# Nightmare-n/GD-MAE

Hardware: AMD Instinct MI355X
Metric: MAE pre-train frames/sec (Waymo-shape, 180k pts, 75% mask) (higher is better)
Workload: dtype bf16

## Files before the change

gd-mae_amd/csrc/decoder_blocks.hip:

```cpp
#include "../../include/gdmae_hip.h"
#include "common.h"
#include "dw_grouped.h"
#include <stdlib.h>

typedef float f32x16 __attribute__((ext_vector_type(16)));
typedef __bf16 bf16x8 __attribute__((ext_vector_type(8)));
typedef short s16x4 __attribute__((ext_vector_type(4)));

namespace {

constexpr int kC = 128;
constexpr int kChunk = 64;
constexpr int kXBytes = kChunk * kC * 2;
constexpr int kMaxTok = 2048;
constexpr int kHP = 6;
constexpr int kQ = 32;

template <int U>
struct Geo {
  static constexpr int TPC = kChunk / (U * U);
  static constexpr int HW = U + 2;
  static constexpr int HS = HW * HW;
  static constexpr int LT = U == 4 ? 36 : 24;
  static constexpr int NP = 2;
// ... 259 lines not shown

template <int U>
int block_dw_launch(const BlockDwArgs& A, hipStream_t st) {
  using G = Geo<U>;
  constexpr int lds = 2 * G::Buf + 3 * kC * 4 + kMaxTok * 16 + 3 * G::HRP * 4;
  static bool once = false;
  if (!once) {
    GD_CHECK(hipFuncSetAttribute((const void*)k_decoder_block_dw<U>, hipFuncAttributeMaxDynamicSharedMemorySize, lds));
    once = true;
  }
  hipLaunchKernelGGL((k_decoder_block_dw<U>), dim3(4u * (unsigned)A.S), dim3(512), lds, st, A);
  GD_LAUNCH_CHECK();
  return 0;
}

}

extern "C" size_t gdmae_decoder_block_dw_workspace_bytes(long long n, int u) {
  if (u != 2 && u != 4) return 0;
  if (n <= 0) return 256;
  int S = 0, cps = 0;
  block_dw_pick(n, &S, &cps);
  if (!block_dw_fits(u, cps)) return 0;
  return gd_align((size_t)S * 9 * kC * kC * sizeof(float));
}

extern "C" int gdmae_decoder_block_dw(const void* P, const float* a, const float* b, const void* bg, const int* site, long long n, int u,
                                      const void* dYc, const int* tile_slot, int H, int W, float* out, int ld_out, int m_off,
                                      void* workspace, void* stream) {
  GD_REQUIRE(u == 2 || u == 4, "decoder_block_dw: u must be 2 or 4");
// ... 18 lines not shown
```

gd-mae_amd/csrc/plan.hip:

```cpp
#include "../../include/gdmae_hip.h"
#include "common.h"
#include <string.h>

int gd_voxelize_impl(const float* points, long long n_points, int n_cols, const float* lo, const float* vs, const int* grid_xyz,
                     int batch_size, float* points_out, long long* point_coords, long long* inverse, int* inverse32,
                     long long* voxel_coords, int* pillar_cell, int* pillar_pt_off, int* pillar_pts, int* point_rank,
                     int* sample_pillar_off, float* pillar_mean, int* cell2pillar_out, int* counts, void* workspace, size_t workspace_bytes,
                     void* lb_state, float* points_pm, int* row_pillar, hipStream_t st);
size_t gd_voxelize_lb_state_bytes(long long n_points, long long cells);
size_t gd_plan_scan_state_bytes(long long n);
size_t gd_plan_win_state_bytes(long long n);
int gd_plan_visible_tokens(const float* mask, const int* cell2pillar, long long n_cells, int* tok_pillar, int* tok_cell, int* map,
                           int* n_tok, void* lb_state, hipStream_t st);
int gd_plan_downsample(const int* map_in, int B, int Yi, int Xi, int* tok_cell_out, int* map_out, int* n_out, void* lb_state,
                       hipStream_t st);
struct Dims {
  int B, Y, X;
};
struct PlanJob {
  const int* n_tok;
  const int* tok_cell;
  Dims dt, dm;
  const int* map;
  int mode, s;
// ... 176 lines not shown
    O.s[i].win_ws = L.add(name("win_ws"), gd_plan_windows_ws_bytes(B, g.Y, g.X, p->win_x[i], p->win_y[i]));
    const long long wcap = g.n_win < g.cap ? g.n_win : g.cap;
    for (int sh = 0; sh < 2; ++sh)
      for (int k = 0; k < 7; ++k) {
        snprintf(nm, sizeof(nm), "s%d.w%d.%s", i, sh, kWin[k]);
        O.s[i].w[sh][k] = L.add(nm, sizeof(int) * (k < 5 ? g.cap : wcap));
      }
  }
  O.dec_slot = O.dec_list = O.dec_flag = -1;
  if (O.dec) {
    O.dec_slot = L.add("dec.tile_slot", sizeof(int) * nt);
    O.dec_list = L.add("dec.tile_list", sizeof(int) * nt);
    O.dec_flag = L.add("dec.flag", sizeof(int) * nt);
    for (int g = 0; g < p->n_dec; ++g) {
      const StageGeo& sg = O.geo[p->dec_sources[g]];
      snprintf(nm, sizeof(nm), "dec.nbr%d", g);
      O.dec_nbr[g] = L.add(nm, sizeof(int) * sg.cap * sg.up_s * sg.up_s * 9);
    }
  }
  GD_REQUIRE(L.ok, "geometry plan: buffer table too small");
  if (total) *total = L.off;
  if (n_entries) *n_entries = L.n;
  return 0;
}

}

extern "C" int gdmae_geometry_plan_layout(const gdmae_plan_params* p, gdmae_plan_buffer* table, int max_entries, int* n_entries,
                                          size_t* total_bytes) {
  Offsets O;
// ... 89 lines not shown
    rc = gd_plan_windows_all(W, ns, st);
    if (rc) return rc;
  }
  if (O.dec) {
    const int* maps[3];
    int ups[3];
    for (int g = 0; g < p->n_dec; ++g) {
      maps[g] = I(O.s[p->dec_sources[g]].map);
      ups[g] = O.geo[p->dec_sources[g]].up_s;
    }
    int rc = gd_decoder_tiles_lb(maps, ups, p->n_dec, B, gy, gx, I(O.dec_slot), I(O.dec_list), n_act, I(O.dec_flag), lb, st);
    if (rc) return rc;
    for (int g = 0; g < p->n_dec; ++g) {
      const int si = p->dec_sources[g];
      const StageGeo& sg = O.geo[si];
      const int* sites = sg.up_s > 1 ? I(O.s[si].up_sites) : I(O.s[si].tok_cell);
      rc = gd_decoder_site_rulebook(sites, n_tok + si, sg.up_s * sg.up_s, sg.cap * sg.up_s * sg.up_s, I(O.dec_slot), gy, gx, I(O.dec_nbr[g]), st);
      if (rc) return rc;
    }
  }
  return 0;
}
```

gd-mae_amd/gdmae_hip/decoder.py:

```python
from __future__ import annotations

import os
from collections import namedtuple
from dataclasses import dataclass
from types import SimpleNamespace
from typing import Optional

import torch
import torch.nn.functional as F

from . import bn as gbn
from . import lib as L
from . import ops, packing
from . import plan as gplan
from . import timing

CONV_BWD = os.environ.get("GDMAE_DEC_BWD", "implicit")
BLOCK_BWD = os.environ.get("GDMAE_DEC_BLOCK", "1")



def colstats(x2d: torch.Tensor):
    R, C = x2d.shape
    assert x2d.is_contiguous() and x2d.dtype in (torch.float32, torch.bfloat16)
    out = torch.empty(2 * C, dtype=torch.float64, device=x2d.device)
    ws = torch.empty(L.load().gdmae_colstats_workspace_bytes(C), dtype=torch.uint8, device=x2d.device)
    L.call("gdmae_colstats", L.ptr(x2d), R, C, int(x2d.dtype == torch.bfloat16), L.ptr(out), L.ptr(ws), L.stream())
    return out[:C], out[C:]


def _gather_slice(table2d, idx, col0, ncol):
    es = table2d.element_size()
    out = torch.empty(idx.numel(), ncol, dtype=table2d.dtype, device=table2d.device)
# ... 123 lines not shown
    return _Forward(y2, yrows, stats2, ab2, mv2, Z, None, None, bgz)


def _backward_schedule(geom, conv_w, sites, Ps, widths, fwd):
    C2 = fwd.y2.shape[1]
    native = conv_w.dtype == torch.float32 and conv_w.is_contiguous() and C2 % 8 == 0
    tc = geom.tile_conv
    if not (CONV_BWD == "implicit" and fwd.tile_slot is not None and fwd.y2.dtype == torch.bfloat16 and native and C2 == 128
            and all(w == 128 for w in widths) and tc is not None):
        return native, ["taps"] * len(widths)
    stage_bwd = []
    for P, st, u in zip(Ps, sites, tc.ups):
        n, u = P.shape[0], int(u)
        block = (BLOCK_BWD != "0" and u in (2, 4) and P.dtype == torch.bfloat16 and P.is_contiguous() and st.numel() >= n
                 and int(L.load().gdmae_decoder_block_dw_workspace_bytes(n, u)) > 0)
        stage_bwd.append("block" if block else "rulebook")
    return native, stage_bwd


def _save(ctx, **named):
    ctx.saved_names = [(name, len(v) if isinstance(v, (list, tuple)) else None) for name, v in named.items()]
    ctx.save_for_backward(*[t for v in named.values() for t in (v if isinstance(v, (list, tuple)) else (v,))])


def _saved(ctx) -> SimpleNamespace:
    sv, out, j = ctx.saved_tensors, SimpleNamespace(), 0
    for name, n in ctx.saved_names:
        setattr(out, name, sv[j] if n is None else sv[j:j + n])
        j += 1 if n is None else n
    return out

# ... 50 lines not shown
    tot = torch.einsum('ko,koi->i', S, Wk.double()).contiguous()
    dWk = (S[:, :, None] * bgz.double()[None, None, :]).to(torch.promote_types(torch.float32, conv_w.dtype))
    Wd = Wk.to(cdt)
    return S, tot, dWk, Wd


def _stage_dx_spconv(b, i, col):
    n, w, C2 = b.Ps[i].shape[0], b.widths[i], b.y2.shape[1]
    nbr = b.tiles.nbr[i]
    assert nbr.shape[0] == n, (nbr.shape, n)
    dX = torch.empty(n, w, dtype=b.cdt, device=b.y2.device)
    L.call("gdmae_spconv", L.ptr(b.dYc), 0, L.ptr(nbr), b.packed.data_ptr() + i * 9 * w * C2 * 2, n, C2, w, L.ptr(dX), 8, L.stream())
    return dX


def _stage_grads_block(b, i, col):
    dX = _stage_dx_spconv(b, i, col)
    P, ab, w, u = b.Ps[i], b.ab_l[i], b.widths[i], int(b.ups[i])
    n = P.shape[0]
    ws = torch.empty(int(L.load().gdmae_decoder_block_dw_workspace_bytes(n, u)), dtype=torch.uint8, device=P.device)
    L.call("gdmae_decoder_block_dw", L.ptr(P), L.ptr(ab), L.ptr(ab[w:]), L.ptr(b.bgz[col:col + w]), L.ptr(b.sites[i]), n, u, L.ptr(b.dYc),
           L.ptr(b.tile_slot), b.H, b.W, L.ptr(b.dWk), b.bgz.numel(), col, L.ptr(ws), L.stream())
    return dX, None


def _stage_grads_rulebook(b, i, col):
    dX = _stage_dx_spconv(b, i, col)
    P, ab, w, C2 = b.Ps[i], b.ab_l[i], b.widths[i], b.y2.shape[1]
    n = P.shape[0]
    n_pad = int(L.load().gdmae_tap_dw_rows(n, w, C2))
    Zd = torch.empty(n_pad, w, dtype=b.cdt, device=P.device)
    L.call("gdmae_rows_affine_relu_sub", L.ptr(P), _bf(P), None, n, w, L.ptr(ab), L.ptr(ab[w:]), L.ptr(b.bgz[col:col + w]), L.ptr(Zd),
           _bf(Zd), w, 0, L.stream())
    ws = torch.empty(L.load().gdmae_tap_dw_workspace_bytes(n, w, C2), dtype=torch.uint8, device=P.device)
    L.call("gdmae_tap_dw", L.ptr(Zd), n, n_pad, w, L.ptr(b.dYc), L.ptr(b.tiles.nbr[i]), C2, L.ptr(b.dWk), b.bgz.numel(), col, L.ptr(ws),
           L.stream())
    return dX, None

# ... 4 lines not shown
    G = torch.empty(n, 9 * C2, dtype=cdt, device=dev)
    with timing.kernel("k_conv_grad_taps", 2.0 * n * 9 * C2 * G.element_size()):
        L.call("gdmae_conv3x3_grad_taps", L.ptr(b.y2), _bf(b.y2), L.ptr(b.tile_slot), L.ptr(b.ybg), L.ptr(b.k01), L.ptr(b.k01[C2:]),
               L.ptr(b.rows), L.ptr(b.cell2pillar), L.ptr(b.sites[i]), n, b.H, b.W, C2, L.ptr(G), L.stream())
    dX = ops.mm(G, b.Wd[:, :, col:col + w].reshape(9 * C2, w))
    bg = b.bgz[col:col + w]
    if b.Z is not None:
        Zd = _gather_slice(b.Z, b.sites[i], col, w) - bg
    else:
        Zd = torch.empty(n, w, dtype=cdt, device=dev)
        L.call("gdmae_rows_affine_relu_sub", L.ptr(P), _bf(P), None, n, w, L.ptr(ab), L.ptr(ab[w:]), L.ptr(bg), L.ptr(Zd),
               _bf(Zd), w, 0, L.stream())
    return dX, ops.splitk_tn(G, Zd)


_STAGE_GRADS = {"block": _stage_grads_block, "rulebook": _stage_grads_rulebook, "taps": _stage_grads_taps}


def _stage_bn_backward(b, i, col, dX, R, direct):
    P, ab, w = b.Ps[i], b.ab_l[i], b.widths[i]
    n = P.shape[0]
    ws = torch.empty(L.load().gdmae_rows_bwd_stats_workspace_bytes(w), dtype=torch.uint8, device=P.device)
    L.call("gdmae_rows_bwd_stats", L.ptr(P), _bf(P), None, n, w, L.ptr(ab), L.ptr(ab[w:]), L.ptr(dX), _bf(dX), w, 0,
           None, L.ptr(ws), L.stream())
    dgamma, dbeta, c01 = gbn.bwd_coeffs((ws, L.load().gdmae_rows_bwd_stats_rows(n)), 3, b.stats_l[i], ab, b.gammas[i], R,
                                        b.tot[col:col + w], direct)
    dP = torch.empty_like(P)
    L.call("gdmae_rows_bwd", L.ptr(P), _bf(P), None, n, w, L.ptr(ab), L.ptr(ab[w:]), L.ptr(c01), L.ptr(c01[w:]), L.ptr(dX),
           _bf(dX), w, 0, L.ptr(dP), _bf(dP), L.stream())
    return dP, dgamma, dbeta

# ... 41 lines not shown
        B, H, W = geom.B, geom.H, geom.W
        R, k = B * H * W, len(widths)
        b = _saved(ctx)
        b.H, b.W, b.cdt, b.widths = H, W, geom.cdt, widths
        b.rows, st2, b.k01, dgamma2, dbeta2 = _bn2_backward(b, dout, R, ctx.direct[k])
        reg = _region_sums(b, b.rows, B, H, W)
        tap_region, cnt = _region_consts(reg.device, B, H, W)
        algebra = region_algebra_native if ctx.native_region else region_algebra_torch
        S, b.tot, b.dWk, b.Wd = algebra(b.stats2, b.ab2, st2, b.k01, reg, tap_region, cnt, R, b.conv_w, b.bgz, geom.cdt)
        if stage_bwd[0] != "taps":
            b.packed = packing.decoder_conv_packed(ctx.conv_param, widths, ctx.direct_w is not None)
            if b.packed is None:
                stage_bwd = ["taps"] * k
            else:
                b.tiles, b.ups = geom.tile_conv.tiles, geom.tile_conv.ups
                if b.tiles.nbr is None:
                    b.tiles.nbr = gplan.decoder_site_rulebooks(b.tiles, b.sites, b.ups)
                C2 = b.y2.shape[1]
                b.dYc = torch.empty_like(b.y2)
                L.call("gdmae_decoder_dy", L.ptr(b.y2), L.ptr(b.tiles.tile_list), b.tiles.n_act, L.ptr(b.k01), L.ptr(b.k01[C2:]),
                       L.ptr(b.rows), L.ptr(b.cell2pillar), H, W, C2, L.ptr(b.dYc), L.stream())
        grads = [None] * 8
        dW_rows = []
        col = 0
        for i, w in enumerate(widths):
            dX, dW = _STAGE_GRADS[stage_bwd[i]](b, i, col)
            if dW is not None:
                dW_rows.append(dW)
            grads += [None, *_stage_bn_backward(b, i, col, dX, R, ctx.direct[i])]
            col += w
        dWk = b.dWk
        if dW_rows:
# ... 170 lines not shown
```

gd-mae_amd/gdmae_hip/lib.py:

```python
from __future__ import annotations

import ctypes as C
import os

import torch

_HERE = os.path.dirname(os.path.abspath(__file__))
LIB_PATH = os.path.abspath(os.path.join(_HERE, "..", "csrc", "libgdmae_hip.so"))
if os.environ.get("GDMAE_LIB"):
    LIB_PATH = os.path.abspath(os.environ["GDMAE_LIB"])


class GdmaeHipError(RuntimeError):
    pass


_P, _I, _L, _F, _D, _Z = C.c_void_p, C.c_int, C.c_longlong, C.c_float, C.c_double, C.c_size_t

SIGNATURES = {
    "gdmae_abi_version": (_I, []),
    "gdmae_target_arch": (C.c_char_p, []),
    "gdmae_last_error": (C.c_char_p, []),
    "gdmae_voxelize_workspace_bytes": (_Z, [_L, _I, _I, _I, _I]),
    "gdmae_voxelize": (_I, [_P, _L, _I, _P, _P, _P, _I, _P, _P, _P, _P, _P, _P, _P, _P, _P, _P, _P, _P, _P, _P, _Z, _P]),
# ... 94 lines not shown
    "gdmae_gemm_tn_splitk": (_I, [_P, _P, _P, _L, _I, _I, _I, _I, _P, _P]),
    "gdmae_conv_block_scratch_bytes": (_Z, [_L, _L, _I, _I, _I]),
    "gdmae_spconv_packed_bytes": (_Z, [_I, _I]),
    "gdmae_spconv_pack_jobs": (_I, [_P, _I, _I, _I, _P, _P]),
    "gdmae_spconv": (_I, [_P, _I, _P, _P, _L, _I, _I, _P, _I, _P]),
    "gdmae_spconv_bias_relu": (_I, [_P, _I, _P, _P, _P, _L, _I, _I, _P, _P]),
    "gdmae_spconv_stat_rows": (_I, [_I, _I, _I]),
    "gdmae_spconv_stats": (_I, [_P, _I, _P, _P, _L, _I, _I, _P, _P, _P]),
    "gdmae_decoder_dy": (_I, [_P, _P, _I, _P, _P, _P, _P, _I, _I, _I, _P, _P]),
    "gdmae_decoder_site_rulebook": (_I, [_P, _P, _I, _L, _P, _I, _I, _P, _P]),
    "gdmae_tap_dw_rows": (_L, [_L, _I, _I]),
    "gdmae_tap_dw_workspace_bytes": (_Z, [_L, _I, _I]),
    "gdmae_tap_dw": (_I, [_P, _L, _L, _I, _P, _P, _I, _P, _I, _I, _P, _P]),
    "gdmae_decoder_block_dw_workspace_bytes": (_Z, [_L, _I]),
    "gdmae_decoder_block_dw": (_I, [_P, _P, _P, _P, _P, _L, _I, _P, _P, _I, _I, _P, _I, _I, _P, _P]),
    "gdmae_conv_block_fwd": (_I, [_P, _P]),
    "gdmae_conv_block_bwd": (_I, [_P, _P]),
    "gdmae_encoder_layer_bytes": (_I, [_L, _I, _I, _I, _I, _P, _P, _P]),
    "gdmae_dw_gemm_workspace_bytes": (_Z, [_L, _I, _I]),
    "gdmae_dw_gemm": (_I, [_P, _P, _L, _I, _I, _P, _P, _P, _P]),
    "gdmae_layer_packed_bytes": (_Z, [_I, _I]),
    "gdmae_layer_pack_jobs": (_I, [_P, _P, _P, _P, _I, _I, _P, _P]),
    "gdmae_layer_pack_job_count": (_I, [_I, _I]),
    "gdmae_tok_gemm_pack": (_I, [_P, _I, _P]),
    "gdmae_tok_gemm": (_I, [_P, _P, _P, _L, _L, _I, _I, _I, _P, _P, _P, _P, _P, _P, _F, _P, _P, _P, _P, _P, _P, _P]),
    "gdmae_tok_gemm_qkv": (_I, [_P, _P, _P, _P, _P, _L, _I, _P, _P, _P]),
    "gdmae_tok_gemm_ffn": (_I, [_P, _P, _P, _P, _P, _L, _L, _I, _P, _P, _P, _P, _F, _P, _P, _P, _P, _P, _P, _P, _P]),
    "gdmae_tok_gemm_ln_bwd_rows": (_I, [_I]),
    "gdmae_tok_gemm_ln_bwd": (_I, [_P, _P, _L, _L, _I, _I, _P, _P, _P, _P, _P, _P, _P, _P, _P, _P]),
    "gdmae_encoder_layer_fwd": (_I, [_P, _P]),
# ... 69 lines not shown
}

class LayerArgs(C.Structure):
    _fields_ = ([("n", _L), ("d", _I), ("ff", _I), ("nhead", _I), ("bf16", _I), ("eps", _F), ("tau_min", _F), ("n_levels", _I),
                 ("n_win", _I * 4), ("max_tokens", _I * 4)]
                + [(k, _P) for k in ("tok_pos", "csr_tok", "win_start", "win_len", "pos_table", "Win", "bin", "Wo", "bo", "W1", "b1",
                                     "W2", "b2", "g1", "be1", "g2", "be2", "tau", "x", "y", "dy", "dx", "dWin", "dbin", "dtau", "dWo",
                                     "dbo", "dW1", "db1", "dW2", "db2", "dg1", "dbe1", "dg2", "dbe2", "saved", "scratch", "packed")]
                + [("x_bf16", _I), ("res_out", _P), ("dres", _P), ("dx_bf16", _P), ("path", _I)])


class PlanParams(C.Structure):
    _fields_ = [("n_points", _L), ("n_cols", _I), ("batch_size", _I), ("lo", _F * 3), ("vs", _F * 3), ("grid", _I * 3), ("n_stages", _I),
                ("stride", _I * 4), ("win_x", _I * 4), ("win_y", _I * 4), ("n_levels", _I * 4), ("drop_lo", (_I * 3) * 4),
                ("drop_hi", (_I * 3) * 4), ("max_tokens", (_I * 3) * 4), ("masked", _I), ("keep_frac", _D), ("n_dec", _I),
                ("dec_sources", _I * 4), ("want_pm", _I), ("cap_points", _L)]


class PlanBuffer(C.Structure):
    _fields_ = [("name", C.c_char * 40), ("offset", _L), ("bytes", _L)]


class ConvBlockArgs(C.Structure):
    _fields_ = ([("n_in", _L), ("n_out", _L), ("cin", _I), ("cout", _I), ("bf16", _I), ("x_f32", _I), ("g_f32", _I),
                 ("eps", _F), ("momentum", _F)]
                + [(k, _P) for k in ("x", "nbr", "nbr_t", "W", "gamma", "beta", "running_mean", "running_var", "num_batches", "cols",
                                     "y", "stats", "ab", "mv", "out", "g", "dx", "dW", "dgamma", "dbeta", "scratch", "packed_fwd", "packed_bwd")]
                + [("out_f32", _I)])


_lib = None
# ... 65 lines not shown
```

gd-mae_amd/gdmae_hip/plan.py:

```python
from __future__ import annotations

from dataclasses import dataclass, field
from typing import List, Optional

import torch

from . import lib as L

I32 = torch.int32


def _empty(n, dtype, dev):
    return torch.empty(int(n), dtype=dtype, device=dev)


@dataclass
class VoxelPlan:
    batch_size: int
    grid: tuple
    lo: tuple
    vs: tuple
    n_cols: int
    N: int
    M: int
# ... 149 lines not shown
    sources = tuple(int(v) for v in sources)
    dt = ep.dec_tiles
    if dt is not None and dt.sources == sources and dt.H == H and dt.W == W:
        return dt
    st = [ep.stages[i] for i in sources]
    B = st[0].B
    ups = [H // sp.Y for sp in st]
    assert all(sp.Y * u == H and sp.X * u == W for sp, u in zip(st, ups))
    r = _decoder_tiles_launch([sp.map for sp in st], ups, B, H, W, st[0].map.device)
    n = int(r["n_act"].item())
    ep.dec_tiles = DecoderTiles(sources, B, H, W, n, r["tile_slot"], r["tile_list"][:n])
    ep.dec_tiles.nbr = _site_rulebooks(ep.dec_tiles, st, ups)
    return ep.dec_tiles


def decoder_site_rulebooks(dt: "DecoderTiles", sites, ups, n_tok=None):
    out = []
    for g, (st, u) in enumerate(zip(sites, ups)):
        n_dev = torch.tensor([st.numel() // (u * u) if n_tok is None else n_tok[g]], dtype=I32, device=st.device)
        nbr = _empty(st.numel() * 9, I32, st.device)
        L.call("gdmae_decoder_site_rulebook", L.ptr(st.contiguous()), L.ptr(n_dev), u * u, st.numel(), L.ptr(dt.tile_slot), dt.H, dt.W,
               L.ptr(nbr), L.stream())
        out.append(nbr.view(-1, 9))
    return out


def _site_rulebooks(dt: "DecoderTiles", stages, ups):
    sites = (sp.tok_cell if u == 1 else (sp._up_sites[1] if getattr(sp, "_up_sites", None) is not None and sp._up_sites[0] == u
                                         else upsample_cells(sp.tok_cell, sp.Y, sp.X, u).reshape(-1).contiguous())
             for sp, u in zip(stages, ups))
    return decoder_site_rulebooks(dt, sites, ups, [sp.n_tok for sp in stages])


def _encoder_launch(vox, m_cap: int, strides, window_shapes, drop_infos, keep_frac, noise, dec_sources=None) -> dict:
    if isinstance(vox, dict):
        dev, grid, B = vox["src"].device, vox["grid"], vox["batch_size"]
        sample_off, pillar_cell, vcounts = vox["sample_off"], vox["pillar_cell"], vox["counts"]
    else:
        dev, grid, B = vox.points.device, vox.grid, vox.batch_size
# ... 123 lines not shown
    e = _encoder_launch(vox, vox.M, strides, window_shapes, drop_infos, keep_frac, noise, dec_sources)
    return _encoder_finalize(e, e["counts"].tolist(), vox.M)


import collections
import time as _time

EVENT_WAIT_S = 0.0

_PLAN_SHAPES = collections.OrderedDict()
_PLAN_SHAPES_MAX = 32
_PLAN_GRANULE = 16384
_PINNED = {}


def _plan_shape(n0, ncols, B, pcr, voxel_size, grid_size, strides, window_shapes, drop_infos, keep_frac, dec_sources):
    gx, gy, gz = (int(g) for g in grid_size)
    lo = tuple(float(v) for v in pcr[:3])
    vs = tuple(float(v) for v in voxel_size)
    drops = tuple(tuple(map(tuple, _drop_arrays(d))) for d in drop_infos)
    n_exact = n0
    n0 = max(1, (n0 + _PLAN_GRANULE - 1) // _PLAN_GRANULE) * _PLAN_GRANULE
    key = (n0, ncols, B, lo, vs, (gx, gy, gz), tuple(int(s) for s in strides), tuple(tuple(int(v) for v in w) for w in window_shapes),
           drops, None if keep_frac is None else float(keep_frac), None if dec_sources is None else tuple(int(i) for i in dec_sources))
    hit = _PLAN_SHAPES.get(key)
    if hit is not None:
        _PLAN_SHAPES.move_to_end(key)
        return hit
    del n_exact
    import ctypes as C
    ns = len(strides)
    assert gz == 1, "the SST backbone works on single-layer pillar grids (spt_backbone_mae.py:94)"
    assert 1 <= ns <= 4
    P = L.PlanParams()
    P.n_points, P.cap_points, P.n_cols, P.batch_size = n0, n0, ncols, B
    for i in range(3):
        P.lo[i], P.vs[i] = lo[i], vs[i]
        P.grid[i] = (gx, gy, gz)[i]
    P.n_stages = ns
# ... 10 lines not shown
        for l in range(len(dT)):
            P.drop_lo[i][l], P.drop_hi[i][l], P.max_tokens[i][l] = dlo[l], dhi[l], dT[l]
        cap_in = cap
        if int(strides[i]) > 1:
            assert int(strides[i]) == 2, "only the k3 s2 p1 strided sparse conv of the shipped configs is implemented"
            Y, X = (Y - 1) // 2 + 1, (X - 1) // 2 + 1
            cap = min(4 * cap, B * Y * X)
        us = gy // Y
        up_s = us if (us >= 1 and us * Y == gy and us * X == gx) else 0
        geo.append(dict(Y=Y, X=X, cap=cap, cap_in=cap_in, up_s=up_s, strided=int(strides[i]) > 1, T=list(dT)))
    P.masked = int(keep_frac is not None)
    P.keep_frac = float(keep_frac) if keep_frac is not None else 1.0
    P.n_dec = 0 if dec_sources is None else len(dec_sources)
    for g in range(P.n_dec):
        P.dec_sources[g] = int(dec_sources[g])
    P.want_pm = 1
    table = (L.PlanBuffer * 160)()
    n_ent, total = C.c_int(0), C.c_size_t(0)
    L.call("gdmae_geometry_plan_layout", C.byref(P), table, 160, C.byref(n_ent), C.byref(total))
    names = {table[i].name.decode(): (int(table[i].offset), int(table[i].bytes)) for i in range(n_ent.value)}
    hit = _PLAN_SHAPES[key] = (P, names, int(total.value), geo, m_cap, (lo, vs, (gx, gy, gz)))
    while len(_PLAN_SHAPES) > _PLAN_SHAPES_MAX:
        _PLAN_SHAPES.popitem(last=False)
    return hit


class _Arena:

    def __init__(self, raw, names):
        self.raw, self.names = raw, names
# ... 6 lines not shown
        off, _ = self.names[name]
        es = 8 if dtype == torch.int64 else 4
        strides, acc = [], 1
        for d in reversed(shape):
            strides.append(acc)
            acc *= int(d)
        return self.base[dtype].as_strided(tuple(int(d) for d in shape), tuple(reversed(strides)), off // es)


class PlanPrefetch:

    _side = {}
    _arena_bytes = {}

    def __init__(self, points, point_cloud_range, voxel_size, grid_size, batch_size, strides, window_shapes, drop_infos,
                 keep_frac=None, noise=None, ready=None, dec_sources=None):
        import ctypes as C
        assert points.is_cuda and points.dtype == torch.float32 and points.dim() == 2
        points = points.contiguous()
        dev = points.device
        main = torch.cuda.current_stream(dev)
        side = PlanPrefetch._side.setdefault(dev.index, torch.cuda.Stream(device=dev))
        side.wait_stream(main)
        if ready is not None:
            side.wait_event(ready)
        points.record_stream(side)
        if noise is not None:
            noise.record_stream(side)
        n0, ncols = points.shape
        P, names, total, geo, m_cap, _ = self.shape = _plan_shape(n0, ncols, int(batch_size), point_cloud_range, voxel_size, grid_size,
                                                                    strides, window_shapes, drop_infos, keep_frac, dec_sources)
        self.masked, self.dec_sources, self.batch_size, self.ncols = keep_frac is not None, dec_sources, int(batch_size), ncols
        with torch.cuda.stream(side):
            cap = PlanPrefetch._arena_bytes.get(dev.index, 0)
            if total > cap:
                cap = PlanPrefetch._arena_bytes[dev.index] = -(-total // (64 << 20)) * (64 << 20)
            raw = torch.empty(cap, dtype=torch.uint8, device=dev)
            if self.masked and noise is None:
                noise = torch.rand(m_cap, device=dev, dtype=torch.float32)
            if noise is not None:
                assert noise.dtype == torch.float32 and noise.numel() >= 1
                noise = noise.contiguous()
            Pc = L.PlanParams.from_buffer_copy(P)
            Pc.n_points = n0
            L.call("gdmae_geometry_plan", C.byref(Pc), L.ptr(points), None if noise is None else L.ptr(noise), L.ptr(raw), total, L.stream())
            self.arena = _Arena(raw, names)
# ... 47 lines not shown
                wpre = f"{pre}w{k}."
                wps.append(WindowPlan(V(wpre + "tok_win", i32, n), V(wpre + "tok_level", i32, n), V(wpre + "tok_slot", i32, n),
                                      V(wpre + "tok_pos", i32, n), V(wpre + "csr_tok", i32, n), V(wpre + "win_start", i32, nw),
                                      V(wpre + "win_len", i32, nw), [int(v) for v in wc[0:3]], [int(v) for v in wc[3:6]], list(g["T"])))
            n_prev = (int(c[2 + i - 1]) if i > 0 else n_vis) if g["strided"] else 0
            sp = StagePlan(B, g["Y"], g["X"], n, V(pre + "tok_cell", i32, n), V(pre + "map", i32, B * g["Y"] * g["X"]),
                           V(pre + "nbr_subm", i32, n, 9), V(pre + "nbr_down", i32, n, 9) if g["strided"] else None,
                           V(pre + "nbr_down_t", i32, n_prev, 9) if g["strided"] else None, wps)
            sp._nbr_subm_t = V(pre + "nbr_subm_t", i32, n, 9)
            sp._up_sites = (g["up_s"], V(pre + "up_sites", i32, n * g["up_s"] * g["up_s"])) if g["up_s"] > 1 else None
            stages.append(sp)
        dt = None
        if A.has("dec.tile_slot"):
            n_act = int(c[2 + ns + 16 * ns])
            nt = B * ((gy + 7) // 8) * ((gx + 7) // 8)
            nbrs = [V(f"dec.nbr{g}", i32, stages[int(si)].n_tok * geo[int(si)]["up_s"] ** 2, 9) for g, si in enumerate(self.dec_sources)]
            dt = DecoderTiles(tuple(int(i) for i in self.dec_sources), B, gy, gx, n_act, V("dec.tile_slot", i32, nt), V("dec.tile_list", i32, n_act),
                              nbrs)
        ep = EncoderPlan(V("mask", f32, M) if self.masked else None, V("tok_pillar", i32, stages[0].n_tok if not geo[0]["strided"] else n_vis),
                         stages, dt)
        self.arena = self.points = self.keep = None
        return vox, ep


def _tensors_of(obj):
    out = []
    if isinstance(obj, torch.Tensor):
        if obj.is_cuda:
            out.append(obj)
    elif isinstance(obj, dict):
        for v in obj.values():
# ... 6 lines not shown
```

gd-mae_amd/pcdet/models/backbones_3d/spt_backbone_mae.py:

```python
import torch
import torch.nn as nn

from .spt_backbone import SSTBlockV1, build_decoder, run_decoder, stage_plan_args
from ...utils.spconv_utils import SparseConvTensor
from gdmae_hip import decoder as gdec, ops, plan as gplan


def _only_the_pred_head_sees_the_gradient(pred) -> bool:
    fn = pred.grad_fn
    if fn is None or not type(fn).__name__.startswith('ViewBackward') or pred._backward_hooks or pred.retains_grad:
        return False
    nxt = [f for f, _ in fn.next_functions if f is not None]
    if len(nxt) != 1 or 'PredHeadFn' not in type(nxt[0]).__name__:
        return False
    return not getattr(nxt[0], '_tensor_pre_hooks', None) and not getattr(nxt[0], '_pre_hooks', None) and not getattr(nxt[0], '_retains_grad_hooks', None)


class _DeferredPlan:
    __slots__ = ("_mod", "_args", "_pf")

    def __init__(self, mod, args):
        self._mod, self._args, self._pf = mod, args, None

    def __call__(self):
# ... 75 lines not shown
                                              pre_conv_hook=hook)
        else:
            sf = run_decoder(self.model_cfg, self.decoder_deblocks, self.decoder_conv_out, hidden)
            assert sf.shape[0] == B and sf.shape[2] == Y and sf.shape[3] == X
            pyramid = ops.GatherUnique.apply(sf.permute(0, 2, 3, 1).reshape(B * Y * X, sf.shape[1]), vox.pillar_cell)
        src0 = self.model_cfg.FEATURES_SOURCE[0]
        batch_dict.update({'encoded_spconv_tensor': hidden[-1], 'encoded_spconv_tensor_stride': Y0 // hidden[-1].spatial_shape[0],
                           'multi_scale_3d_features': feats, 'multi_scale_3d_strides': strides, 'spatial_features': sf,
                           'spatial_features_stride': strides[src0] // self.model_cfg.FUSE_LAYER[src0].UPSAMPLE_STRIDE})
        batch_dict.update({'voxel_features': pyramid, 'voxel_coords': all_coords,
                           'voxel_shuffle_inds': torch.arange(all_coords.shape[0], device=all_coords.device)})
        self.forward_ret_dict = self.target_assigner(batch_dict)
        return batch_dict

    def prefetch_plan(self, points, batch_size, noise=None, ready=None):
        return gplan.PlanPrefetch(points, self.point_cloud_range, self.voxel_size, self.grid_size, int(batch_size),
                                  *stage_plan_args(self.model_cfg.SST_BLOCK_LIST), keep_frac=1 - self.mask_ratio, noise=noise,
                                  ready=ready, dec_sources=self._dec_sources())

    def prefetch_plan_under_decoder(self, points, batch_size, noise=None, ready=None):
        self._pre_conv_hook = d = _DeferredPlan(self, (points, batch_size, noise, ready))
        return d

    def _dec_sources(self):
        if self.decoder_impl != 'sparse' or self.decoder_conv_impl != 'tiles':
            return None
        return [int(src[-1]) - 1 for src in self.model_cfg.FEATURES_SOURCE]

    def target_assigner(self, batch_dict):
        vox = batch_dict['_gdmae_vox']
        gt = ops.group_gt_points(vox, self.mask_cfg.NUM_GT_POINTS)
        flat = gdec.pred_head(batch_dict['voxel_features'], self.decoder_pred)
        return {'pred_points': flat.view(vox.M, -1, 3), 'gt_points': gt, 'mask': batch_dict['voxel_mae_mask'],
# ... 2 lines not shown
```

include/gdmae_hip.h:

```cpp
#ifndef GDMAE_HIP_H
#define GDMAE_HIP_H

#include <stddef.h>
#include <stdint.h>

#ifdef __cplusplus
extern "C" {
#endif

int gdmae_abi_version(void);
const char* gdmae_target_arch(void);
const char* gdmae_last_error(void);

size_t gdmae_voxelize_workspace_bytes(long long n_points, int batch_size, int gx, int gy, int gz);
int gdmae_voxelize(const float* points, long long n_points, int n_cols, const float* lo, const float* vs,
                   const int* grid_xyz, int batch_size, float* points_out, long long* point_coords,
                   long long* inverse, int* inverse32, long long* voxel_coords, int* pillar_cell,
                   int* pillar_pt_off, int* pillar_pts, int* point_rank, int* sample_pillar_off,
                   float* pillar_mean, int* cell2pillar, int* counts, void* workspace, size_t workspace_bytes,
                   void* stream);

int gdmae_decorate_points(const float* points, const long long* point_coords, const int* inverse32,
                          const float* pillar_mean, long long N, int n_cols, const float* lo, const float* vs,
                          float* out, void* stream);
// ... 222 lines not shown
int gdmae_spconv_stat_rows(int cin, int cout, int x_f32);
int gdmae_spconv_stats(const void* X, int x_f32, const int* nbr, const void* packed, long long n, int cin, int cout, void* Y, float* part,
                       void* stream);
int gdmae_decoder_dy(const void* Yc, const int* tile_list, int n_act, const float* k0, const float* k1, const float* rows,
                     const int* cell2pillar, int H, int W, int C, void* dYc, void* stream);
int gdmae_decoder_site_rulebook(const int* site, const int* n_dev, int sites_per_tok, long long cap_sites, const int* tile_slot,
                                int H, int W, int* nbr, void* stream);
long long gdmae_tap_dw_rows(long long n, int M, int N);
size_t gdmae_tap_dw_workspace_bytes(long long n, int M, int N);
int gdmae_tap_dw(const void* G, long long n, long long n_pad, int M, const void* X, const int* nbr, int N, float* out, int ld_out,
                 int m_off, void* workspace, void* stream);
size_t gdmae_decoder_block_dw_workspace_bytes(long long n, int u);
int gdmae_decoder_block_dw(const void* P, const float* a, const float* b, const void* bg, const int* site, long long n, int u,
                           const void* dYc, const int* tile_slot, int H, int W, float* out, int ld_out, int m_off, void* workspace,
                           void* stream);
int gdmae_conv_block_fwd(const gdmae_conv_block_args* args , void* stream);
int gdmae_conv_block_bwd(const gdmae_conv_block_args* args , void* stream);

typedef struct gdmae_layer_args {
  long long n;
  int d, ff, nhead, bf16;
  float eps, tau_min;
  int n_levels;
  int n_win[4], max_tokens[4];
  const int* tok_pos;
  const int* csr_tok;
  const int* win_start;
  const int* win_len;
  const float* pos_table;
  const void *Win, *bin, *Wo, *bo, *W1, *b1, *W2, *b2;
// ... 110 lines not shown
  long long n_points;
  int n_cols, batch_size;
  float lo[3], vs[3];
  int grid[3];
  int n_stages;
  int stride[GDMAE_PLAN_MAX_STAGES];
  int win_x[GDMAE_PLAN_MAX_STAGES], win_y[GDMAE_PLAN_MAX_STAGES];
  int n_levels[GDMAE_PLAN_MAX_STAGES];
  int drop_lo[GDMAE_PLAN_MAX_STAGES][3], drop_hi[GDMAE_PLAN_MAX_STAGES][3], max_tokens[GDMAE_PLAN_MAX_STAGES][3];
  int masked;
  double keep_frac;
  int n_dec;
  int dec_sources[GDMAE_PLAN_MAX_STAGES];
  int want_pm;
  long long cap_points;
} gdmae_plan_params;
typedef struct gdmae_plan_buffer {
  char name[40];
  long long offset, bytes;
} gdmae_plan_buffer;
int gdmae_geometry_plan_layout(const gdmae_plan_params* p, gdmae_plan_buffer* table, int max_entries, int* n_entries,
                               size_t* total_bytes);
int gdmae_geometry_plan(const gdmae_plan_params* p, const float* points, const float* noise, void* arena, size_t arena_bytes,
                        void* stream);

size_t gdmae_center_head_targets_workspace_bytes(int B, int num_max_objs);
int gdmae_center_head_targets(const float* gt_boxes, int B, int n_max, int box_dim, const int* class_map, int n_class_total,
                              int n_cls, const float* pc_range , const float* voxel_size ,
                              float feature_map_stride, int fw, int fh, int num_max_objs, double gaussian_overlap, int min_radius,
                              float* heatmap, float* ret_boxes, long long* inds, long long* mask, void* workspace, void* stream);
// ... 109 lines not shown
```

Baseline: 1104.

## Add block-tiled decoder conv dX kernel and skip unneeded site rulebooks

Adds a new HIP kernel that computes the decoder 3x3 conv input gradient per block of tokens. It stages a halo of dY rows from the tile map into swizzled LDS and runs bf16 MFMA over the 9 taps, replacing the gather-based spconv dX path. Because this path no longer needs the per-site neighbour rulebook, the geometry plan can now skip building and allocating those rulebooks for u=2/4 stages. The trade-offs are halo reads of masked rows, tied to fixed tile shapes, and more plan-key complexity.

```diff
diff --git a/gd-mae_amd/csrc/decoder_blocks.hip b/gd-mae_amd/csrc/decoder_blocks.hip
--- a/gd-mae_amd/csrc/decoder_blocks.hip
+++ b/gd-mae_amd/csrc/decoder_blocks.hip
@@ -297,6 +297,217 @@
   return 0;
 }
 
+struct BlockDxArgs {
+  const unsigned short* dY;
+  const int* site;
+  const int* tile_slot;
+  const uint4* Wp;
+  unsigned short* dZ;
+  long long n;
+  int ntok, H, W, TH, TW;
+};
+
+union DxFrag {
+  uint4 q;
+  bf16x8 v;
+};
+
+template <int U>
+__device__ __forceinline__ int dx_swz(int tl, int hy, int hx) {
+  return U == 4 ? (((hy & 3) << 2) | (hx & 3)) : (((tl & 3) << 2) | ((hy & 1) << 1) | (hx & 1));
+}
+
+template <int U, int ROWS, int WAVES>
+__global__ __launch_bounds__(64 * WAVES, 2) void k_decoder_block_dx(BlockDxArgs A) {
+  constexpr int NTHR = 64 * WAVES;
+  constexpr int KS = kC / 16;
+  constexpr int MB = kC / 32;
+  constexpr int WPB = WAVES / MB;
+  constexpr int NPW = ROWS / 32 / WPB;
+  constexpr int HW = U + 2, HS = HW * HW;
+  constexpr int NT = ROWS / (U * U);
+  constexpr int NHR = NT * HS;
+  constexpr int NP = NHR * 16 / NTHR;
+  constexpr int NR = (NHR + NTHR - 1) / NTHR;
+  constexpr int SP = kC * 2 + 16;
+  static_assert(WPB >= 1 && NPW >= 1 && NPW * WPB * 32 == ROWS && NP * NTHR == NHR * 16 && ROWS * SP <= NHR * 256, "tile shape");
+  constexpr int RING = KS;
+  extern __shared__ __align__(16) unsigned char lds[];
+  int* rowidx = reinterpret_cast<int*>(lds + NHR * 256);
+  const int tid = threadIdx.x, lane = tid & 63, wv = tid >> 6;
+  const long long row0 = (long long)blockIdx.x * ROWS;
+  const long long tok0 = (long long)blockIdx.x * NT;
+  const int mb0 = wv / WPB;
+  const int nb0 = (wv % WPB) * NPW;
+
+  int sv[NR];
+#pragma unroll
+  for (int j = 0; j < NR; ++j) {
+    const int hr = tid + j * NTHR < NHR ? tid + j * NTHR : NHR - 1;
+    const long long tok = tok0 + hr / HS;
+    sv[j] = A.site[(tok < A.ntok ? tok : (long long)A.ntok - 1) * (U * U)];
+  }
+
+  const uint4* __restrict__ wp = A.Wp + (size_t)mb0 * 64 + lane;
+  DxFrag wr[RING];
+#pragma unroll
+  for (int ks = 0; ks < RING; ++ks) wr[ks].q = wp[(size_t)ks * MB * 64];
+
+  {
+    int slot[NR], loc[NR];
+#pragma unroll
+    for (int j = 0; j < NR; ++j) {
+      const int hr = tid + j * NTHR < NHR ? tid + j * NTHR : NHR - 1;
+      const int tl = hr / HS, rem = hr - tl * HS;
+      const int hy = rem / HW, hx = rem - hy * HW;
+      const int x0 = sv[j] % A.W, r = sv[j] / A.W;
+      const int y0 = r % A.H, bb = r / A.H;
+      const int yy = y0 + hy - 1, xx = x0 + hx - 1;
+      const bool in = tok0 + tl < A.ntok && yy >= 0 && yy < A.H && xx >= 0 && xx < A.W;
+      slot[j] = A.tile_slot[in ? (bb * A.TH + (yy >> 3)) * A.TW + (xx >> 3) : 0];
+      loc[j] = in ? (yy & 7) * 8 + (xx & 7) : -1;
+    }
+#pragma unroll
+    for (int j = 0; j < NR; ++j) {
+      const int hr = tid + j * NTHR < NHR ? tid + j * NTHR : NHR - 1;
+      rowidx[hr] = (loc[j] >= 0 && slot[j] >= 0) ? slot[j] * 64 + loc[j] : -1;
+    }
+  }
+  __syncthreads();
+
+  {
+    const int pc = tid & 15;
+    uint4 q[NP];
+    unsigned keep = 0u;
+#pragma unroll
+    for (int p = 0; p < NP; ++p) {
+      const int rix = rowidx[(p * NTHR + tid) >> 4];
+      const bool ok = rix >= 0;
+      keep |= ok ? 1u << p : 0u;
+      q[p] = *reinterpret_cast<const uint4*>(A.dY + (long long)(ok ? rix : 0) * kC + pc * 8);
+    }
+#pragma unroll
+    for (int p = 0; p < NP; ++p) {
+      const int hr = (p * NTHR + tid) >> 4;
+      const int tl = hr / HS, rem = hr - tl * HS;
+      const int hy = rem / HW, hx = rem - hy * HW;
+      const unsigned m = ((keep >> p) & 1u) ? 0xFFFFFFFFu : 0u;
+      uint4 v = q[p];
+      v.x &= m; v.y &= m; v.z &= m; v.w &= m;
+      *reinterpret_cast<uint4*>(lds + hr * 256 + ((pc ^ dx_swz<U>(tl, hy, hx)) << 4)) = v;
+    }
+  }
+  __syncthreads();
+
+  int tlb[NPW], hyc[NPW], hxc[NPW];
+#pragma unroll
+  for (int b = 0; b < NPW; ++b) {
+    const int r = (nb0 + b) * 32 + (lane & 31);
+    tlb[b] = r / (U * U);
+    hyc[b] = (r / U) % U + 1;
+    hxc[b] = r % U + 1;
+  }
+  const int hsel = lane >> 5;
+
+  f32x16 acc[NPW];
+#pragma unroll
+  for (int b = 0; b < NPW; ++b)
+#pragma unroll
+    for (int i = 0; i < 16; ++i) acc[b][i] = 0.f;
+
+  int rb[NPW], sw[NPW];
+  auto tap_rows = [&](int tap) {
+#pragma unroll
+    for (int b = 0; b < NPW; ++b) {
+      const int hy = hyc[b] + 1 - tap / 3, hx = hxc[b] + 1 - tap % 3;
+      rb[b] = (tlb[b] * HS + hy * HW + hx) * 256;
+      sw[b] = (dx_swz<U>(tlb[b], hy, hx) ^ hsel) << 4;
+    }
+  };
+  DxFrag sf[2][NPW];
+  tap_rows(0);
+#pragma unroll
+  for (int b = 0; b < NPW; ++b) sf[0][b].q = *reinterpret_cast<const uint4*>(lds + rb[b] + sw[b]);
+#pragma unroll
+  for (int tap = 0; tap < 9; ++tap) {
+#pragma unroll
+    for (int ks = 0; ks < KS; ++ks) {
+      const int g = tap * KS + ks;
+      if (ks + 1 < KS) {
+#pragma unroll
+        for (int b = 0; b < NPW; ++b) sf[(g + 1) & 1][b].q = *reinterpret_cast<const uint4*>(lds + rb[b] + (((ks + 1) * 32) ^ sw[b]));
+      } else if (tap < 8) {
+        tap_rows(tap + 1);
+#pragma unroll
+        for (int b = 0; b < NPW; ++b) sf[(g + 1) & 1][b].q = *reinterpret_cast<const uint4*>(lds + rb[b] + sw[b]);
+      }
+#pragma unroll
+      for (int b = 0; b < NPW; ++b) acc[b] = __builtin_amdgcn_mfma_f32_32x32x16_bf16(wr[g % RING].v, sf[g & 1][b].v, acc[b], 0, 0, 0);
+      if (g + RING < 9 * KS) wr[g % RING].q = wp[(size_t)(g + RING) * MB * 64];
+      __builtin_amdgcn_sched_barrier(0);
+    }
+  }
+  __syncthreads();
+
+  {
+    const int cb = mb0 * 32 + 4 * (lane >> 5);
+#pragma unroll
+    for (int b = 0; b < NPW; ++b) {
+      const int row = (nb0 + b) * 32 + (lane & 31);
+#pragma unroll
+      for (int q = 0; q < 4; ++q) {
+        uint2 o;
+        o.x = gd_pack_bf16(acc[b][4 * q], acc[b][4 * q + 1]);
+        o.y = gd_pack_bf16(acc[b][4 * q + 2], acc[b][4 * q + 3]);
+        *reinterpret_cast<uint2*>(lds + row * SP + (cb + 8 * q) * 2) = o;
+      }
+    }
+  }
+  __syncthreads();
+  {
+    constexpr int OCPR = kC / 8;
+    constexpr int ORPP = NTHR / OCPR;
+    const int c = tid % OCPR, r = tid / OCPR;
+#pragma unroll
+    for (int p = 0; p < ROWS / ORPP; ++p) {
+      const int rl = p * ORPP + r;
+      if (row0 + rl < A.n) *reinterpret_cast<uint4*>(A.dZ + (row0 + rl) * kC + c * 8) = *reinterpret_cast<const uint4*>(lds + rl * SP + c * 16);
+    }
+  }
+}
+
+template <int U, int ROWS, int WAVES>
+int block_dx_launch(const BlockDxArgs& A, hipStream_t st) {
+  constexpr int nhr = ROWS / (U * U) * (U + 2) * (U + 2);
+  constexpr int lds = nhr * 256 + nhr * 4;
+  static bool once = false;
+  if (!once) {
+    GD_CHECK(hipFuncSetAttribute((const void*)k_decoder_block_dx<U, ROWS, WAVES>, hipFuncAttributeMaxDynamicSharedMemorySize, lds));
+    once = true;
+  }
+  hipLaunchKernelGGL((k_decoder_block_dx<U, ROWS, WAVES>), dim3((unsigned)gd_div_up(A.n, ROWS)), dim3(64 * WAVES), lds, st, A);
+  GD_LAUNCH_CHECK();
+  return 0;
+}
+
+}
+
+extern "C" int gdmae_decoder_block_dx_supported(long long n, int u) {
+  return (u == 2 || u == 4) && n >= 0 && n % (u * u) == 0 && n < (1ll << 31);
+}
+
+extern "C" int gdmae_decoder_block_dx(const void* dYc, const int* site, long long n, int u, const int* tile_slot, int H, int W,
+                                      const void* packed, void* dZ, void* stream) {
+  GD_REQUIRE(u == 2 || u == 4, "decoder_block_dx: u must be 2 or 4");
+  GD_REQUIRE(n >= 0 && n % (u * u) == 0, "decoder_block_dx: rows must be whole tokens (u * u sites each)");
+  if (n == 0) return 0;
+  GD_REQUIRE(n < (1ll << 31) && H > 0 && W > 0 && H % u == 0 && W % u == 0, "decoder_block_dx: map size");
+  hipStream_t st = (hipStream_t)stream;
+  BlockDxArgs A{(const unsigned short*)dYc, site, tile_slot, (const uint4*)packed, (unsigned short*)dZ, n, (int)(n / (u * u)), H, W,
+                (H + 7) / 8, (W + 7) / 8};
+  GdTimed timed(GD_T_DEC_CONV_BWD, st, (double)n / (u * u) * ((u + 2) * (u + 2) * 2.0 * kC + 4.0) + (double)n * 2.0 * kC + 18.0 * kC * kC,
+                2.0 * n * 9.0 * kC * kC);
+  return u == 4 ? block_dx_launch<4, 128, 4>(A, st) : block_dx_launch<2, 64, 4>(A, st);
 }
 
 extern "C" size_t gdmae_decoder_block_dw_workspace_bytes(long long n, int u) {
diff --git a/gd-mae_amd/csrc/plan.hip b/gd-mae_amd/csrc/plan.hip
--- a/gd-mae_amd/csrc/plan.hip
+++ b/gd-mae_amd/csrc/plan.hip
@@ -214,6 +214,8 @@
     O.dec_flag = L.add("dec.flag", sizeof(int) * nt);
     for (int g = 0; g < p->n_dec; ++g) {
       const StageGeo& sg = O.geo[p->dec_sources[g]];
+      O.dec_nbr[g] = -1;
+      if (p->dec_skip_rulebook[g]) continue;
       snprintf(nm, sizeof(nm), "dec.nbr%d", g);
       O.dec_nbr[g] = L.add(nm, sizeof(int) * sg.cap * sg.up_s * sg.up_s * 9);
     }
@@ -333,6 +335,7 @@
     for (int g = 0; g < p->n_dec; ++g) {
       const int si = p->dec_sources[g];
       const StageGeo& sg = O.geo[si];
+      if (O.dec_nbr[g] < 0) continue;
       const int* sites = sg.up_s > 1 ? I(O.s[si].up_sites) : I(O.s[si].tok_cell);
       rc = gd_decoder_site_rulebook(sites, n_tok + si, sg.up_s * sg.up_s, sg.cap * sg.up_s * sg.up_s, I(O.dec_slot), gy, gx, I(O.dec_nbr[g]), st);
       if (rc) return rc;
diff --git a/gd-mae_amd/gdmae_hip/decoder.py b/gd-mae_amd/gdmae_hip/decoder.py
--- a/gd-mae_amd/gdmae_hip/decoder.py
+++ b/gd-mae_amd/gdmae_hip/decoder.py
@@ -17,6 +17,12 @@
 
 CONV_BWD = os.environ.get("GDMAE_DEC_BWD", "implicit")
 BLOCK_BWD = os.environ.get("GDMAE_DEC_BLOCK", "1")
+BLOCK_DX = os.environ.get("GDMAE_DEC_BLOCK_DX", "1")
+
+
+def plan_rulebooks(ups):
+    blocks = CONV_BWD == "implicit" and BLOCK_BWD != "0" and BLOCK_DX != "0"
+    return [not (blocks and int(u) in (2, 4)) for u in ups]
 
 
 
@@ -170,7 +176,9 @@
         n, u = P.shape[0], int(u)
         block = (BLOCK_BWD != "0" and u in (2, 4) and P.dtype == torch.bfloat16 and P.is_contiguous() and st.numel() >= n
                  and int(L.load().gdmae_decoder_block_dw_workspace_bytes(n, u)) > 0)
-        stage_bwd.append("block" if block else "rulebook")
+        blocks = (block and BLOCK_DX != "0" and st.is_contiguous() and st.dtype == torch.int32
+                  and int(L.load().gdmae_decoder_block_dx_supported(n, u)) == 1)
+        stage_bwd.append("blocks" if blocks else ("block" if block else "rulebook"))
     return native, stage_bwd
 
 
@@ -251,14 +259,29 @@
     return dX
 
 
+def _stage_dx_block(b, i, col):
+    n, w, C2 = b.Ps[i].shape[0], b.widths[i], b.y2.shape[1]
+    dX = torch.empty(n, w, dtype=b.cdt, device=b.y2.device)
+    L.call("gdmae_decoder_block_dx", L.ptr(b.dYc), L.ptr(b.sites[i]), n, int(b.ups[i]), L.ptr(b.tile_slot), b.H, b.W,
+           b.packed.data_ptr() + i * 9 * w * C2 * 2, L.ptr(dX), L.stream())
+    return dX
+
+
+def _stage_grads_blocks(b, i, col):
+    return _stage_dx_block(b, i, col), _stage_dw_block(b, i, col)
+
+
 def _stage_grads_block(b, i, col):
-    dX = _stage_dx_spconv(b, i, col)
+    return _stage_dx_spconv(b, i, col), _stage_dw_block(b, i, col)
+
+
+def _stage_dw_block(b, i, col):
     P, ab, w, u = b.Ps[i], b.ab_l[i], b.widths[i], int(b.ups[i])
     n = P.shape[0]
     ws = torch.empty(int(L.load().gdmae_decoder_block_dw_workspace_bytes(n, u)), dtype=torch.uint8, device=P.device)
     L.call("gdmae_decoder_block_dw", L.ptr(P), L.ptr(ab), L.ptr(ab[w:]), L.ptr(b.bgz[col:col + w]), L.ptr(b.sites[i]), n, u, L.ptr(b.dYc),
            L.ptr(b.tile_slot), b.H, b.W, L.ptr(b.dWk), b.bgz.numel(), col, L.ptr(ws), L.stream())
-    return dX, None
+    return None
 
 
 def _stage_grads_rulebook(b, i, col):
@@ -293,7 +316,7 @@
     return dX, ops.splitk_tn(G, Zd)
 
 
-_STAGE_GRADS = {"block": _stage_grads_block, "rulebook": _stage_grads_rulebook, "taps": _stage_grads_taps}
+_STAGE_GRADS = {"blocks": _stage_grads_blocks, "block": _stage_grads_block, "rulebook": _stage_grads_rulebook, "taps": _stage_grads_taps}
 
 
 def _stage_bn_backward(b, i, col, dX, R, direct):
@@ -365,8 +388,7 @@
                 stage_bwd = ["taps"] * k
             else:
                 b.tiles, b.ups = geom.tile_conv.tiles, geom.tile_conv.ups
-                if b.tiles.nbr is None:
-                    b.tiles.nbr = gplan.decoder_site_rulebooks(b.tiles, b.sites, b.ups)
+                gplan.ensure_site_rulebooks(b.tiles, b.sites, b.ups, [s in ("rulebook", "block") for s in stage_bwd])
                 C2 = b.y2.shape[1]
                 b.dYc = torch.empty_like(b.y2)
                 L.call("gdmae_decoder_dy", L.ptr(b.y2), L.ptr(b.tiles.tile_list), b.tiles.n_act, L.ptr(b.k01), L.ptr(b.k01[C2:]),
diff --git a/gd-mae_amd/gdmae_hip/lib.py b/gd-mae_amd/gdmae_hip/lib.py
--- a/gd-mae_amd/gdmae_hip/lib.py
+++ b/gd-mae_amd/gdmae_hip/lib.py
@@ -132,6 +132,8 @@
     "gdmae_tap_dw": (_I, [_P, _L, _L, _I, _P, _P, _I, _P, _I, _I, _P, _P]),
     "gdmae_decoder_block_dw_workspace_bytes": (_Z, [_L, _I]),
     "gdmae_decoder_block_dw": (_I, [_P, _P, _P, _P, _P, _L, _I, _P, _P, _I, _I, _P, _I, _I, _P, _P]),
+    "gdmae_decoder_block_dx_supported": (_I, [_L, _I]),
+    "gdmae_decoder_block_dx": (_I, [_P, _P, _L, _I, _P, _I, _I, _P, _P, _P]),
     "gdmae_conv_block_fwd": (_I, [_P, _P]),
     "gdmae_conv_block_bwd": (_I, [_P, _P]),
     "gdmae_encoder_layer_bytes": (_I, [_L, _I, _I, _I, _I, _P, _P, _P]),
@@ -231,7 +233,7 @@
     _fields_ = [("n_points", _L), ("n_cols", _I), ("batch_size", _I), ("lo", _F * 3), ("vs", _F * 3), ("grid", _I * 3), ("n_stages", _I),
                 ("stride", _I * 4), ("win_x", _I * 4), ("win_y", _I * 4), ("n_levels", _I * 4), ("drop_lo", (_I * 3) * 4),
                 ("drop_hi", (_I * 3) * 4), ("max_tokens", (_I * 3) * 4), ("masked", _I), ("keep_frac", _D), ("n_dec", _I),
-                ("dec_sources", _I * 4), ("want_pm", _I), ("cap_points", _L)]
+                ("dec_sources", _I * 4), ("want_pm", _I), ("cap_points", _L), ("dec_skip_rulebook", _I * 4)]
 
 
 class PlanBuffer(C.Structure):
diff --git a/gd-mae_amd/gdmae_hip/plan.py b/gd-mae_amd/gdmae_hip/plan.py
--- a/gd-mae_amd/gdmae_hip/plan.py
+++ b/gd-mae_amd/gdmae_hip/plan.py
@@ -187,15 +187,40 @@
     return ep.dec_tiles
 
 
-def decoder_site_rulebooks(dt: "DecoderTiles", sites, ups, n_tok=None):
+def decoder_upsampling(strides, grid_size, dec_sources):
+    gx, gy = int(grid_size[0]), int(grid_size[1])
+    Y, X, ups = gy, gx, []
+    for s in strides:
+        if int(s) > 1:
+            Y, X = (Y - 1) // 2 + 1, (X - 1) // 2 + 1
+        us = gy // Y
+        ups.append(us if (us >= 1 and us * Y == gy and us * X == gx) else 0)
+    return [ups[int(i)] for i in dec_sources]
+
+
+def decoder_site_rulebooks(dt: "DecoderTiles", sites, ups, n_tok=None, which=None):
     out = []
     for g, (st, u) in enumerate(zip(sites, ups)):
+        if which is not None and not which[g]:
+            out.append(None)
+            continue
         n_dev = torch.tensor([st.numel() // (u * u) if n_tok is None else n_tok[g]], dtype=I32, device=st.device)
         nbr = _empty(st.numel() * 9, I32, st.device)
         L.call("gdmae_decoder_site_rulebook", L.ptr(st.contiguous()), L.ptr(n_dev), u * u, st.numel(), L.ptr(dt.tile_slot), dt.H, dt.W,
                L.ptr(nbr), L.stream())
         out.append(nbr.view(-1, 9))
     return out
+
+
+def ensure_site_rulebooks(dt: "DecoderTiles", sites, ups, need):
+    if dt.nbr is None:
+        dt.nbr = [None] * len(ups)
+    missing = [bool(n) and dt.nbr[g] is None for g, n in enumerate(need)]
+    if any(missing):
+        for g, nbr in enumerate(decoder_site_rulebooks(dt, sites, ups, which=missing)):
+            if nbr is not None:
+                dt.nbr[g] = nbr
+    return dt.nbr
 
 
 def _site_rulebooks(dt: "DecoderTiles", stages, ups):
@@ -349,7 +374,7 @@
 _PINNED = {}
 
 
-def _plan_shape(n0, ncols, B, pcr, voxel_size, grid_size, strides, window_shapes, drop_infos, keep_frac, dec_sources):
+def _plan_shape(n0, ncols, B, pcr, voxel_size, grid_size, strides, window_shapes, drop_infos, keep_frac, dec_sources, dec_rulebooks=None):
     gx, gy, gz = (int(g) for g in grid_size)
     lo = tuple(float(v) for v in pcr[:3])
     vs = tuple(float(v) for v in voxel_size)
@@ -357,7 +382,8 @@
     n_exact = n0
     n0 = max(1, (n0 + _PLAN_GRANULE - 1) // _PLAN_GRANULE) * _PLAN_GRANULE
     key = (n0, ncols, B, lo, vs, (gx, gy, gz), tuple(int(s) for s in strides), tuple(tuple(int(v) for v in w) for w in window_shapes),
-           drops, None if keep_frac is None else float(keep_frac), None if dec_sources is None else tuple(int(i) for i in dec_sources))
+           drops, None if keep_frac is None else float(keep_frac), None if dec_sources is None else tuple(int(i) for i in dec_sources),
+           None if dec_rulebooks is None else tuple(bool(v) for v in dec_rulebooks))
     hit = _PLAN_SHAPES.get(key)
     if hit is not None:
         _PLAN_SHAPES.move_to_end(key)
@@ -398,6 +424,7 @@
     P.n_dec = 0 if dec_sources is None else len(dec_sources)
     for g in range(P.n_dec):
         P.dec_sources[g] = int(dec_sources[g])
+        P.dec_skip_rulebook[g] = int(dec_rulebooks is not None and not dec_rulebooks[g])
     P.want_pm = 1
     table = (L.PlanBuffer * 160)()
     n_ent, total = C.c_int(0), C.c_size_t(0)
@@ -434,7 +461,7 @@
     _arena_bytes = {}
 
     def __init__(self, points, point_cloud_range, voxel_size, grid_size, batch_size, strides, window_shapes, drop_infos,
-                 keep_frac=None, noise=None, ready=None, dec_sources=None):
+                 keep_frac=None, noise=None, ready=None, dec_sources=None, dec_rulebooks=None):
         import ctypes as C
         assert points.is_cuda and points.dtype == torch.float32 and points.dim() == 2
         points = points.contiguous()
@@ -449,7 +476,8 @@
             noise.record_stream(side)
         n0, ncols = points.shape
         P, names, total, geo, m_cap, _ = self.shape = _plan_shape(n0, ncols, int(batch_size), point_cloud_range, voxel_size, grid_size,
-                                                                    strides, window_shapes, drop_infos, keep_frac, dec_sources)
+                                                                    strides, window_shapes, drop_infos, keep_frac, dec_sources,
+                                                                    dec_rulebooks if dec_sources is not None else None)
         self.masked, self.dec_sources, self.batch_size, self.ncols = keep_frac is not None, dec_sources, int(batch_size), ncols
         with torch.cuda.stream(side):
             cap = PlanPrefetch._arena_bytes.get(dev.index, 0)
@@ -527,7 +555,8 @@
         if A.has("dec.tile_slot"):
             n_act = int(c[2 + ns + 16 * ns])
             nt = B * ((gy + 7) // 8) * ((gx + 7) // 8)
-            nbrs = [V(f"dec.nbr{g}", i32, stages[int(si)].n_tok * geo[int(si)]["up_s"] ** 2, 9) for g, si in enumerate(self.dec_sources)]
+            nbrs = [V(f"dec.nbr{g}", i32, stages[int(si)].n_tok * geo[int(si)]["up_s"] ** 2, 9) if A.has(f"dec.nbr{g}") else None
+                    for g, si in enumerate(self.dec_sources)]
             dt = DecoderTiles(tuple(int(i) for i in self.dec_sources), B, gy, gx, n_act, V("dec.tile_slot", i32, nt), V("dec.tile_list", i32, n_act),
                               nbrs)
         ep = EncoderPlan(V("mask", f32, M) if self.masked else None, V("tok_pillar", i32, stages[0].n_tok if not geo[0]["strided"] else n_vis),
diff --git a/gd-mae_amd/pcdet/models/backbones_3d/spt_backbone_mae.py b/gd-mae_amd/pcdet/models/backbones_3d/spt_backbone_mae.py
--- a/gd-mae_amd/pcdet/models/backbones_3d/spt_backbone_mae.py
+++ b/gd-mae_amd/pcdet/models/backbones_3d/spt_backbone_mae.py
@@ -113,9 +113,10 @@
         return batch_dict
 
     def prefetch_plan(self, points, batch_size, noise=None, ready=None):
+        args, srcs = stage_plan_args(self.model_cfg.SST_BLOCK_LIST), self._dec_sources()
+        books = None if srcs is None else gdec.plan_rulebooks(gplan.decoder_upsampling(args[0], self.grid_size, srcs))
         return gplan.PlanPrefetch(points, self.point_cloud_range, self.voxel_size, self.grid_size, int(batch_size),
-                                  *stage_plan_args(self.model_cfg.SST_BLOCK_LIST), keep_frac=1 - self.mask_ratio, noise=noise,
-                                  ready=ready, dec_sources=self._dec_sources())
+                                  *args, keep_frac=1 - self.mask_ratio, noise=noise, ready=ready, dec_sources=srcs, dec_rulebooks=books)
 
     def prefetch_plan_under_decoder(self, points, batch_size, noise=None, ready=None):
         self._pre_conv_hook = d = _DeferredPlan(self, (points, batch_size, noise, ready))
diff --git a/include/gdmae_hip.h b/include/gdmae_hip.h
--- a/include/gdmae_hip.h
+++ b/include/gdmae_hip.h
@@ -260,6 +260,9 @@
 int gdmae_decoder_block_dw(const void* P, const float* a, const float* b, const void* bg, const int* site, long long n, int u,
                            const void* dYc, const int* tile_slot, int H, int W, float* out, int ld_out, int m_off, void* workspace,
                            void* stream);
+int gdmae_decoder_block_dx_supported(long long n, int u);
+int gdmae_decoder_block_dx(const void* dYc, const int* site, long long n, int u, const int* tile_slot, int H, int W, const void* packed,
+                           void* dZ, void* stream);
 int gdmae_conv_block_fwd(const gdmae_conv_block_args* args , void* stream);
 int gdmae_conv_block_bwd(const gdmae_conv_block_args* args , void* stream);
 
@@ -400,6 +403,7 @@
   int dec_sources[GDMAE_PLAN_MAX_STAGES];
   int want_pm;
   long long cap_points;
+  int dec_skip_rulebook[GDMAE_PLAN_MAX_STAGES];
 } gdmae_plan_params;
 typedef struct gdmae_plan_buffer {
   char name[40];
```

After: 1109, median of 6. No clear change (+0.5%).
